# DaLi-Jack/G4Splat

Hardware: AMD Instinct MI355X
Metric: rasterized Gaussians/s fwd+bwd @1600x1200 (higher is better)
Workload: dtype f32

## Files before the change

g4splat_amd/csrc/api.hip:

```cpp
#include <stdarg.h>
#include <stdio.h>
#include <stdlib.h>
#include <string.h>

#include <atomic>
#include <mutex>
#include <vector>

#include "g4s_internal.h"

using namespace g4s;

extern "C" int g4s_knn_launch_internal(int P, const float* points, float* meanDists, char* workspace, hipStream_t s);
extern "C" void g4s_maps_launch_internal(int fwd, int W, int H, float depth_ratio, const float* allmap, const float* wvt,
                                         const float* fpt, float* cam, float* const* outs, const float* surf_depth_in,
                                         const float* const* grads, float* g_allmap, hipStream_t s);

namespace {
thread_local char t_err[512] = "";
}

namespace g4s {
void clear_error() { t_err[0] = 0; }
int fail(int code, const char* fmt, ...) {
// ... 459 lines not shown
}

extern "C" int g4s_rasterizer_forward_presized(
    char* geom_buffer, size_t geom_bytes, char* binning_buffer, size_t binning_bytes, char* image_buffer, size_t image_bytes,
    int instance_capacity, uint32_t* status_dev, int P, int D, int M, const float* background, int width, int height,
    const float* means3D, const float* shs, const float* sh_rest, const float* colors_precomp, const float* opacities,
    const float* scales, float scale_modifier, const float* rotations, const float* transMat_precomp,
    const float* viewmatrix, const float* projmatrix, const float* cam_pos, float tan_fovx, float tan_fovy,
    float* out_color, float* out_others, int* radii, int debug, void* stream) {
    t_err[0] = 0;
    if (instance_capacity < 0 || !status_dev) return fail(G4S_ERR_INVALID_ARGUMENT, "capacity must be >= 0 and status_dev non-NULL");
    if (!geom_buffer || !binning_buffer || !image_buffer) return fail(G4S_ERR_INVALID_ARGUMENT, "state buffers must not be NULL");
    FixedChunk g{geom_buffer, geom_bytes}, b{binning_buffer, binning_bytes}, im{image_buffer, image_bytes};
    DECLARE_FORWARD_CALL(c);
    c.capacity = instance_capacity; c.status_dev = status_dev;
    c.geometry = {fixed_chunk_cb, &g}; c.binning = {fixed_chunk_cb, &b}; c.image = {fixed_chunk_cb, &im};
    c.shs = shs; c.shs_rest = M > 1 ? sh_rest : nullptr; c.colors_precomp = colors_precomp;
    const int rc = rasterizer_forward_impl(c);
    return rc < 0 ? rc : G4S_OK;
}

extern "C" size_t g4s_rasterizer_backward_workspace(int P, int R) {
    (void)P;
    return align_up((size_t)(R > 0 ? R : 1) * GRAD_STRIDE * 4) + 256;
}

static int rasterizer_backward_impl(const BackwardCall& c) {
    hipStream_t stream = (hipStream_t)c.stream;
    const int P = c.P, M = c.M, R = c.R, debug = c.debug;
    t_err[0] = 0;
    if (P < 0 || R < 0 || c.width <= 0 || c.height <= 0) return fail(G4S_ERR_INVALID_ARGUMENT, "bad sizes");
    if (P == 0) return G4S_OK;
    if (!c.geom_buffer || !c.image_buffer || (R > 0 && !c.binning_buffer))
        return fail(G4S_ERR_INVALID_ARGUMENT, "state buffers must not be NULL");
    if (!c.dL_dpix || !c.dL_depths || !c.dL_dmean2D || !c.dL_dopacity || !c.dL_dcolor || !c.dL_dmean3D ||
        !c.dL_dscale || !c.dL_drot || (M > 0 && !c.dL_dsh) || (c.shs_rest && M > 1 && !c.dL_dsh_rest))
        return fail(G4S_ERR_INVALID_ARGUMENT, "NULL gradient pointer");
    if (c.workspace_bytes < g4s_rasterizer_backward_workspace(P, R) || !c.workspace)
        return fail(G4S_ERR_INVALID_ARGUMENT, "workspace too small");
    if (misaligned(c.rotations, 16) || misaligned(c.scales, 8) || misaligned(c.dL_drot, 16) || misaligned(c.dL_dscale, 8))
        return fail(G4S_ERR_INVALID_ARGUMENT, "rotations/dL_drot must be 16-byte, scales/dL_dscale 8-byte aligned");

    const FrameGeom FG = frame_geom(c.width, c.height);
    const int tiles = FG.tiles;
    const GeomLayout GL = geom_layout((size_t)P);
    const BinLayout BL = bin_layout((size_t)R);
    const ImgLayout IL = img_layout((size_t)c.width * c.height, (size_t)tiles);
    char* geom = align_ptr(c.geom_buffer);
    char* img = align_ptr(c.image_buffer);
    const float* rec = (const float*)(geom + GL.rec);
    const int* const radii = c.radii ? c.radii : (const int*)(geom + GL.internal_radii);
    float* grad_inst = (float*)align_ptr(c.workspace);

    uint32_t* hot_count = (uint32_t*)(img + IL.hot_count);
    uint32_t* hot_list = (uint32_t*)(img + IL.hot_list);
    uint8_t* rec_flag = nullptr;
    bool sh_prezeroed = false;
    if (R > 0) {
        char* bin = align_ptr(c.binning_buffer);
        rec_flag = (uint8_t*)(bin + BL.rec_flag);
        BlendBwdArgs bb{};
        bb.W = c.width; bb.H = c.height; bb.tiles_x = FG.tiles_x; bb.tiles_y = FG.tiles_y;
        bb.ranges = (const uint32_t*)(img + IL.ranges);
        uint32_t* tile_order_bwd = (uint32_t*)(img + IL.tile_order_bwd);
        launch_tile_order(tiles, (const uint32_t*)(img + IL.tile_depth), tile_order_bwd, stream, hot_count);
        bb.tile_order = opt(OPT_BWD_FWD_ORDER) ? (const uint32_t*)(img + IL.tile_order) : tile_order_bwd;
        bb.entries = (const uint64_t*)(bin + (FG.entries_in_b ? BL.ent_b : BL.ent_a));
        bb.rec = rec; bb.bg = c.background;
        bb.final_T = (const float*)(img + IL.final_T);
        bb.n_contrib = (const uint32_t*)(img + IL.n_contrib);
        bb.qhit = (const uint8_t*)(bin + BL.qhit);
        bb.dL_dpix = c.dL_dpix; bb.dL_depths = c.dL_depths; bb.grad_inst = grad_inst; bb.rec_flag = rec_flag;
        bb.n_slots = (uint32_t)R;
        const long long avg_list = (long long)R / (tiles > 0 ? tiles : 1);
        const long long outlier = 4 * avg_list > BWD_HOT_THRESHOLD ? 4 * avg_list : BWD_HOT_THRESHOLD;
        const int hot_override = opt(OPT_BWD_HOT_THRESHOLD);
        bb.hot_threshold = hot_override != G4S_OPTION_UNSET ? hot_override
                           : (tiles <= BWD_FOUR_WAVE_MAX_TILES ? -1 : (int)(outlier < 0x7fffffff ? outlier : 0x7fffffff));
        bb.hot_count = hot_count; bb.hot_list = hot_list;
        if (bb.hot_threshold >= 0 && M > 0 && !opt(OPT_NO_SIDE_ZERO) && !c.accumulate) {
            float* zb[2] = {c.dL_dsh, c.dL_dsh_rest};
            const size_t zn[2] = {(size_t)P * (c.dL_dsh_rest ? 1 : M) * 3, c.dL_dsh_rest ? (size_t)P * (M - 1) * 3 : 0};
            bool ok = true;
            for (int z = 0; z < 2; z++) ok = ok && (zn[z] == 0 || (!misaligned(zb[z], 16) && (zn[z] >> 2) < 0x80000000ull));
            if (ok) {
                for (int z = 0; z < 2; z++) {
                    if (zn[z] == 0) continue;
                    bb.zero_base[z] = zb[z]; bb.zero_quads[z] = (uint32_t)(zn[z] >> 2); bb.zero_tail[z] = (uint32_t)(zn[z] & 3);
                }
                sh_prezeroed = true;
            }
        }
        { ProfScope ps(PF_BLEND_BWD, stream); launch_blend_bwd(bb, stream); }
        CHECK_LAUNCH("blend_bwd");
    }

    const float focal_y = c.height / (2.0f * c.tan_fovy);
    const float focal_x = c.width / (2.0f * c.tan_fovx);
    PreprocessBwdArgs pb{};
    pb.P = P; pb.D = c.D; pb.M = M;
    pb.W = (int)(focal_x * c.tan_fovx * 2);
    pb.H = (int)(focal_y * c.tan_fovy * 2);
    pb.means3D = c.means3D; pb.scales = c.scales; pb.rotations = c.rotations; pb.shs = c.shs;
    pb.transMat_precomp = c.transMat_precomp; pb.colors_precomp = c.colors_precomp;
    pb.viewmatrix = c.viewmatrix; pb.projmatrix = c.projmatrix; pb.campos = c.campos;
    pb.radii = radii; pb.rec = rec; pb.clamped = (const uint8_t*)(geom + GL.clamped); pb.grad_inst = grad_inst;
    pb.rec_flag = rec_flag; pb.n_slots = (uint32_t)R;
    pb.frame_W = c.width; pb.frame_H = c.height; pb.scale_modifier = c.scale_modifier;
    pb.shs_rest = c.shs_rest; pb.dL_dsh_rest = c.dL_dsh_rest; pb.sh_prezeroed = sh_prezeroed;
    pb.accumulate = c.accumulate;
    pb.view_stats = c.view_stats;
    const g4s_packed_rows* const packed = c.packed;
    if (packed != nullptr && packed->rows != nullptr) {
        if (c.accumulate) return fail(G4S_ERR_INVALID_ARGUMENT, "packed rows: only the first view of a batch (first_view != 0) can write them");
        if (!packed->block_offs || packed->capacity < 0 || c.shs == nullptr)
            return fail(G4S_ERR_INVALID_ARGUMENT, "packed rows: block_offs must not be NULL, capacity >= 0, colours from SH");
        pb.packed_rows = packed->rows; pb.packed_block_offs = packed->block_offs;
        pb.packed_capacity = (uint32_t)(packed->capacity < 0xFFFFFFFFll ? packed->capacity : 0xFFFFFFFFll);
    }
    if (c.after_event) HIP_TRY(hipStreamWaitEvent(stream, (hipEvent_t)c.after_event, 0));
    pb.sh_vec16 = (c.shs != nullptr && c.shs_rest == nullptr && M == 16 && !misaligned(c.shs, 16) && !misaligned(c.dL_dsh, 16));
    pb.dL_dmean2D = c.dL_dmean2D; pb.dL_dnormal = c.dL_dnormal; pb.dL_dopacity = c.dL_dopacity; pb.dL_dcolor = c.dL_dcolor;
    pb.dL_dmean3D = c.dL_dmean3D; pb.dL_dtransMat = c.dL_dtransMat; pb.dL_dsh = c.dL_dsh; pb.dL_dscale = c.dL_dscale;
    pb.dL_drot = c.dL_drot;
    { ProfScope ps(PF_PREPROCESS_BWD, stream); launch_preprocess_bwd(pb, stream); }
    CHECK_LAUNCH("preprocess_bwd");
    return G4S_OK;
}

extern "C" int g4s_rasterizer_backward(
// ... 407 lines not shown
```

g4splat_amd/csrc/binning.hip:

```cpp
#include "g4s_internal.h"
#include "g4s_device.h"

namespace g4s {


template <typename K>
__device__ __forceinline__ uint32_t radix_digit(K key, uint32_t base, int shift, uint32_t mask) {
    return (uint32_t)((K)(key - (K)base) >> shift) & mask;
}

template <typename K, int ITEMS, int BITS>
__global__ void __launch_bounds__(256) radix_hist_kernel(const K* __restrict__ keys, int n, int shift, uint32_t mask,
                                                         uint32_t* __restrict__ hist, int nblocks,
                                                         const uint32_t* __restrict__ d_n,
                                                         const uint32_t* __restrict__ key_base) {
    constexpr int BINS = 1 << BITS;
    __shared__ uint32_t h[BINS];
    constexpr int TK = 256 * ITEMS;
    const int block = (int)blockIdx.x;
    if (d_n != nullptr) {
        n = (int)*d_n;
        nblocks = (n + TK - 1) / TK;
        if (block >= nblocks) return;
    }
// ... 470 lines not shown
    } else {
#pragma unroll
        for (int k = 0; k < 4; k++) e[k] = entries[i0 + k < R ? i0 + k : R - 1];
    }
    uint32_t prev = i0 > 0 ? entry_tile(entries[i0 - 1]) : 0xFFFFFFFFu;
#pragma unroll
    for (int k = 0; k < 4; k++) {
        const int i = i0 + k;
        if (i >= R) break;
        const uint32_t cur = entry_tile(e[k]);
        if (i == 0) {
            ranges[2 * cur] = 0;
        } else if (cur != prev) {
            ranges[2 * prev + 1] = (uint32_t)i;
            ranges[2 * cur] = (uint32_t)i;
        }
        if (i == R - 1) ranges[2 * cur + 1] = (uint32_t)R;
        prev = cur;
    }
}

constexpr int ORDER_BUCKETS = 2048;
__global__ void __launch_bounds__(1024) tile_order_kernel(int tiles, const uint32_t* __restrict__ ranges,
                                                          uint32_t* __restrict__ order, uint32_t* __restrict__ zero_word) {
    __shared__ uint32_t hist[ORDER_BUCKETS];
    __shared__ uint32_t wsum[16];
    const int t = (int)threadIdx.x;
    if (t == 0 && zero_word != nullptr) *zero_word = 0u;
    for (int i = t; i < ORDER_BUCKETS; i += 1024) hist[i] = 0;
    __syncthreads();
    auto bucket = [](uint32_t n) {
        const uint32_t b = n >> 2;
        return (uint32_t)(ORDER_BUCKETS - 1) - (b < (uint32_t)(ORDER_BUCKETS - 1) ? b : (uint32_t)(ORDER_BUCKETS - 1));
    };
    for (int i = t; i < tiles; i += 1024) atomicAdd(&hist[bucket(ranges[2 * i + 1] - ranges[2 * i])], 1u);
    __syncthreads();
    const uint32_t h0 = hist[2 * t], h1 = hist[2 * t + 1];
    const uint32_t inc = wave_incl_scan_u32(h0 + h1);
    if ((t & 63) == 63) wsum[t >> 6] = inc;
    __syncthreads();
    uint32_t base = 0;
    for (int w = 0; w < (t >> 6); w++) base += wsum[w];
    const uint32_t ex = base + inc - (h0 + h1);
    __syncthreads();
    hist[2 * t] = ex;
    hist[2 * t + 1] = ex + h0;
    __syncthreads();
    for (int i = t; i < tiles; i += 1024) order[atomicAdd(&hist[bucket(ranges[2 * i + 1] - ranges[2 * i])], 1u)] = (uint32_t)i;
}
void launch_tile_order(int tiles, const uint32_t* ranges, uint32_t* tile_order, hipStream_t s, uint32_t* zero_word) {
    hipLaunchKernelGGL(tile_order_kernel, dim3(1), dim3(1024), 0, s, tiles, ranges, tile_order, zero_word);
}

void launch_tile_ranges(int R, const uint64_t* entries, uint32_t* ranges, hipStream_t s, const uint32_t* d_n) {
    if (R <= 0) return;
    hipLaunchKernelGGL(tile_ranges_kernel, dim3((R + 1023) / 1024), dim3(256), 0, s, R, entries, ranges, d_n);
}

}
```

g4splat_amd/csrc/blend.hip:

```cpp
#include "g4s_internal.h"
#include "g4s_device.h"

#ifndef G4S_FWD_PAIRS
#define G4S_FWD_PAIRS 4
#endif

namespace g4s {

__device__ __forceinline__ uint32_t quads_in_box(const float4 q5, uint32_t kx0, uint32_t ky0) {
    const uint32_t x0 = __float_as_uint(q5.x), x1 = __float_as_uint(q5.y), yw = __float_as_uint(q5.w);
    const uint32_t y0 = yw & 0xFFFFu, y1 = yw >> 16;
    const uint32_t cols = (kx0 >= x0 && kx0 <= x1 ? 1u : 0u) | (kx0 + 1 >= x0 && kx0 + 1 <= x1 ? 2u : 0u);
    const uint32_t rows = (ky0 >= y0 && ky0 <= y1 ? 1u : 0u) | (ky0 + 1 >= y0 && ky0 + 1 <= y1 ? 2u : 0u);
    return ((rows & 1u) ? cols : 0u) | ((rows & 2u) ? cols << 2 : 0u);
}

__device__ __forceinline__ bool quad_misses_region(const float4 q0, const float4 q6, const float4 q7, float qx, float qy) {
    const float x1 = qx + 7.0f, y1 = qy + 7.0f;
    const float ddx = fmaxf(fmaxf(qx - q0.x, q0.x - x1), 0.0f), ddy = fmaxf(fmaxf(qy - q0.y, q0.y - y1), 0.0f);
    if (ddx * ddx + ddy * ddy <= q7.z) return false;
    if (q7.x == 0.0f) return false;
    const float ux = q6.z, uy = q6.w, ia = q7.x, ib = q7.y;
    const float ax0 = qx - q6.x, ax1 = x1 - q6.x, ay0 = qy - q6.y, ay1 = y1 - q6.y;
    if (ax0 <= 0.0f && ax1 >= 0.0f && ay0 <= 0.0f && ay1 >= 0.0f) return false;
// ... 202 lines not shown
        a.out_others[pix_id + 3 * N] = st.N1;
        a.out_others[pix_id + 4 * N] = st.N2;
        a.out_others[pix_id + 5 * N] = st.median_depth;
        a.out_others[pix_id + 6 * N] = st.distortion;
    }
}

void launch_blend_fwd(const BlendFwdArgs& a, hipStream_t s) {
    hipLaunchKernelGGL(blend_fwd_kernel, dim3(a.tiles_x * a.tiles_y), dim3(256), 0, s, a);
}


constexpr int BWD_BATCH = 64;

struct BwdPixel {
    float A2, D2, C2, nTfbg;
    uint32_t last_c, median_c;
    float dpx0, dpx1, dpx2, dL_ddepth, dL_daccum, dn0, dn1, dn2, dL_dmedian;
    float T, V_rec, last_dL_dT;
};

__device__ __forceinline__ float fast_rcp(float x) { return __builtin_amdgcn_rcpf(x); }

constexpr int BWD1_BATCH = 48;
struct BwdPixelLite {
    uint32_t last_c;
    float dpx0, dpx1, dpx2, dL_ddepth, dL_daccum, dn0, dn1, dn2;
    float T, V_rec, last_dL_dT;
};
__device__ __forceinline__ void blend_bwd_tile(const BlendBwdArgs& a) {
    __shared__ float4 s_rec[BLEND_QUADS][BWD1_BATCH];
    __shared__ float4 s_cst[256];
    __shared__ float2 s_med[256];

    const int tile = (int)a.tile_order[blockIdx.x];
    const int tile_x = tile % a.tiles_x, tile_y = tile / a.tiles_x;
    const int lane = (int)threadIdx.x;
    const size_t N = (size_t)a.W * a.H;

    const uint32_t r0 = a.ranges[2 * tile], r1 = a.ranges[2 * tile + 1];
    const int n = (int)(r1 - r0);
    if (n == 0) return;

    const int tx0 = tile_x * TILE, ty0 = tile_y * TILE;
    const int px0 = tx0 + (lane & 7), py0 = ty0 + (lane >> 3);
    const float bg0 = a.bg[0], bg1 = a.bg[1], bg2 = a.bg[2];
// ... 22 lines not shown
            x.dn1 = a.dL_depths[pix_id + 3 * N];
            x.dn2 = a.dL_depths[pix_id + 4 * N];
            dL_dmedian = a.dL_depths[pix_id + 5 * N];
            dL_dreg = a.dL_depths[pix_id + 6 * N];
        }
        s_cst[q * 64 + lane] = make_float4((1 - T_final) * dL_dreg, 2.0f * final_D * dL_dreg, final_D2 * dL_dreg,
                                           -T_final * ((bg0 * x.dpx0 + bg1 * x.dpx1) + bg2 * x.dpx2));
        s_med[q * 64 + lane] = make_float2(__uint_as_float(median_c), dL_dmedian);
        x.T = T_final;
        max_last = max(max_last, x.last_c);
    }
    const float mscale = FAR_N / (FAR_N - NEAR_N);
    const float dmd_k = (FAR_N * NEAR_N) / (FAR_N - NEAR_N);
    const bool row_writer = (lane & 15) == 15;
    const int row = lane >> 4;
    const bool lane_b3 = (lane & 8) != 0, lane_b2 = (lane & 4) != 0, quad_writer = (lane & 3) == 0;
    const int term_of_lane = 4 * row + quad_term(lane);

    const int n_live = __builtin_amdgcn_readfirstlane((int)wave_max_u32(max_last));
    if (n_live > a.hot_threshold) {
        if (lane == 0) a.hot_list[atomicAdd(a.hot_count, 1u)] = (uint32_t)tile;
        return;
    }

    for (int hi = n_live; hi > 0; hi -= BWD1_BATCH) {
        const int m = imin_(BWD1_BATCH, hi);
        __syncthreads();
        uint32_t qmask = 0;
        uint32_t slot_l = 0;
        bool nolp_l = false;
        if (lane < m) {
            const uint32_t pos_l = (uint32_t)(hi - 1 - lane);
            qmask = a.qhit[r0 + pos_l];
        }
        if (qmask != 0) {
            const uint32_t pos_l = (uint32_t)(hi - 1 - lane);
            const uint64_t e = a.entries[r0 + pos_l];
            const float4* r = reinterpret_cast<const float4*>(a.rec) + (size_t)entry_idx(e) * REC_QUADS;
            float4 rq[BLEND_QUADS];
#pragma unroll
            for (int i = 0; i < BLEND_QUADS; i++) rq[i] = r[i];
            const float4 q0 = rq[0];
            nolp_l = (__float_as_uint(q0.w) & REC_AFFINE) != 0;
#pragma unroll
            for (int i = 0; i < BLEND_QUADS; i++) s_rec[i][lane] = rq[i];
            slot_l = __float_as_uint(q0.z) + instance_number(__float_as_uint(q0.w), __float_as_uint(reinterpret_cast<const float*>(r)[31]),
// ... 96 lines not shown
                                    dlz = fmaf(dpx_, ky, -(dpy_ * kx));
                        gt0 -= dkx;
                        gt1 -= dky;
                        gt2 -= dkz;
                        gt3 -= dlx;
                        gt4 -= dly;
                        gt5 -= dlz;
                        gt6 += fmaf(pxf, dkx, fmaf(pyf, dlx, dL_dz * e.sx));
                        gt7 += fmaf(pxf, dky, fmaf(pyf, dly, dL_dz * e.sy));
                        gt8 += fmaf(pxf, dkz, fmaf(pyf, dlz, dL_dz));
                    } else {
                        const float c2 = dL_dG * (G * FILTER_INV_SQUARE);
                        glp0 = fmaf(c2, e.dx, glp0);
                        glp1 = fmaf(c2, e.dy, glp1);
                        gt8 += dL_dz;
                        asm volatile("v_mov_b32 %0, 1.0" : "+v"(lowpass));
                    }
                    }
                    gop = fmaf(G, dL_dalpha, gop);
                }
            }
            {
                const uint32_t slot = (uint32_t)__builtin_amdgcn_readlane((int)slot_l, j);
                float t[16] = {gc0, gc1, gc2, gn0, gn1, gn2, gt0, gt1, gt2, gt3, gt4, gt5, gt6, gt7, gt8, gop};
                const float y = wave_sum16_to_quads(t, lane_b3, lane_b2);
                if (slot < a.n_slots) {
                    float* rec = a.grad_inst + (size_t)slot * GRAD_STRIDE;
                    const uint64_t lp_lanes = __ballot(lowpass != 0.0f);
                    uint32_t valid;
                    asm volatile("s_cmp_lg_u64 %1, 0\n\ts_cselect_b32 %0, 3, 1" : "=s"(valid) : "s"(lp_lanes) : "scc");
                    if (quad_writer) {
                        rec[term_of_lane] = y;
                        a.rec_flag[slot] = (uint8_t)valid;
                    }
                    if (valid & 2u) {
                        const float r4 = wave_sum4_to_rows(glp0, glp1, 0.0f, 0.0f);
                        if (row_writer) rec[16 + row] = r4;
                    }
                }
            }
        }
    }
}

__global__ void __launch_bounds__(64) __attribute__((amdgpu_waves_per_eu(4, 4))) blend_bwd_kernel(BlendBwdArgs a) {
    blend_bwd_tile(a);
    const uint32_t lane = threadIdx.x, first = blockIdx.x * 64 + lane, stride = gridDim.x * 64;
#pragma unroll
    for (int z = 0; z < 2; z++) {
        float4* b = reinterpret_cast<float4*>(a.zero_base[z]);
        if (b == nullptr) continue;
        const uint32_t nq = a.zero_quads[z];
        for (uint32_t i = first; i < nq; i += stride) b[i] = make_float4(0.f, 0.f, 0.f, 0.f);
        if (blockIdx.x == 0 && lane < a.zero_tail[z]) reinterpret_cast<float*>(b + nq)[lane] = 0.0f;
    }
}

constexpr int HOT_PART = 20;

__global__ void __launch_bounds__(256) blend_bwd_hot_kernel(BlendBwdArgs a) {
    __shared__ float4 s_rec[BLEND_QUADS][BWD_BATCH];
    __shared__ uint32_t s_slot[BWD_BATCH];
    __shared__ uint32_t s_q[BWD_BATCH];
    __shared__ float s_part[4][BWD_BATCH][HOT_PART];
    __shared__ unsigned long long s_lp[4];
    __shared__ uint32_t s_max[2][4];

    const int wv = (int)(threadIdx.x >> 6), lane = (int)(threadIdx.x & 63);
    const size_t N = (size_t)a.W * a.H;
    const bool all_tiles = a.hot_threshold < 0;
    const uint32_t n_hot = all_tiles ? (uint32_t)(a.tiles_x * a.tiles_y) : *a.hot_count;
    const float bg0 = a.bg[0], bg1 = a.bg[1], bg2 = a.bg[2];
    const float mscale = FAR_N / (FAR_N - NEAR_N);
    const float dmd_k = (FAR_N * NEAR_N) / (FAR_N - NEAR_N);
    const bool row_writer = (lane & 15) == 15;
    const int row = lane >> 4;

    for (uint32_t h = blockIdx.x; h < n_hot; h += gridDim.x) {
        const int tile = (int)(all_tiles ? a.tile_order[h] : a.hot_list[h]);
        const int tile_x = tile % a.tiles_x, tile_y = tile / a.tiles_x;
        const uint32_t r0 = a.ranges[2 * tile];
        const int px = tile_x * TILE + (wv & 1) * 8 + (lane & 7), py = tile_y * TILE + (wv >> 1) * 8 + (lane >> 3);
        const float pxf = (float)px, pyf = (float)py;
        BwdPixel x{};
        {
// ... 10 lines not shown
                x.dpx2 = a.dL_dpix[pix_id + 2 * N];
                x.dL_ddepth = a.dL_depths[pix_id + 0 * N];
                x.dL_daccum = a.dL_depths[pix_id + 1 * N];
                x.dn0 = a.dL_depths[pix_id + 2 * N];
                x.dn1 = a.dL_depths[pix_id + 3 * N];
                x.dn2 = a.dL_depths[pix_id + 4 * N];
                x.dL_dmedian = a.dL_depths[pix_id + 5 * N];
                dL_dreg = a.dL_depths[pix_id + 6 * N];
            }
            x.A2 = (1 - T_final) * dL_dreg;
            x.D2 = 2.0f * final_D * dL_dreg;
            x.C2 = final_D2 * dL_dreg;
            x.nTfbg = -T_final * ((bg0 * x.dpx0 + bg1 * x.dpx1) + bg2 * x.dpx2);
            x.T = T_final;
        }
        __syncthreads();
        {
            const uint32_t ml = wave_max_u32(x.last_c), mm = wave_max_u32(x.median_c);
            if (lane == 0) { s_max[0][wv] = ml; s_max[1][wv] = mm; }
        }
        __syncthreads();
        const int n_live = (int)max(max(s_max[0][0], s_max[0][1]), max(s_max[0][2], s_max[0][3]));
        const uint32_t tile_max_median = max(max(s_max[1][0], s_max[1][1]), max(s_max[1][2], s_max[1][3]));

        for (int hi = n_live; hi > 0; hi -= BWD_BATCH) {
            const int m = imin_(BWD_BATCH, hi);
            __syncthreads();
            if (wv == 0) {
                uint32_t qmask = 0;
                if (lane < m) qmask = a.qhit[r0 + (uint32_t)(hi - 1 - lane)];
                if (qmask != 0) {
                    const uint64_t e = a.entries[r0 + (uint32_t)(hi - 1 - lane)];
                    const float4* r = reinterpret_cast<const float4*>(a.rec) + (size_t)entry_idx(e) * REC_QUADS;
                    float4 rq[BLEND_QUADS];
#pragma unroll
                    for (int i = 0; i < BLEND_QUADS; i++) rq[i] = r[i];
                    if (__float_as_uint(rq[0].w) & REC_AFFINE) qmask |= 16u;
#pragma unroll
                    for (int i = 0; i < BLEND_QUADS; i++) s_rec[i][lane] = rq[i];
                    s_slot[lane] = __float_as_uint(rq[0].z) + instance_number(__float_as_uint(rq[0].w), __float_as_uint(reinterpret_cast<const float*>(r)[31]),
                                                                              (uint32_t)tile_x, (uint32_t)tile_y);
                }
                s_q[lane] = qmask;
            }
            __syncthreads();

            const uint32_t qbits = s_q[lane];
            uint64_t todo = __ballot(((qbits >> wv) & 1u) != 0);
            const uint64_t nolp_mask = __ballot((qbits & 16u) != 0);
            uint64_t lp_mask = 0;
            while (todo) {
                const int j = (int)__builtin_ctzll(todo);
                todo &= ~(1ull << j);
                const bool nolp = (nolp_mask >> j) & 1ull;
                const uint32_t general = (uint32_t)__builtin_amdgcn_readfirstlane(nolp ? 0 : 1);
                const uint32_t pos = (uint32_t)(hi - 1 - j);
                const float4 q0 = s_rec[0][j], q1 = s_rec[1][j], q2 = s_rec[2][j], q3 = s_rec[3][j], q4 = s_rec[4][j];
                float g[18];
#pragma unroll
                for (int i = 0; i < 18; i++) {
                    g[i] = 0.0f;
                    asm volatile("" : "+v"(g[i]));
                }
                bool lowpass = false;
                PairEval e;
                const bool pass = eval_pair(nolp, pxf, pyf, q0.x, q0.y, q2.x, q2.y, q2.z, q2.w, q3.x, q3.y, q3.z, q3.w, q4.x, q1.w, e);
// ... 63 lines not shown
                    }
                    }
                    g[15] = fmaf(G, dL_dalpha, g[15]);
                }
                float t[16] = {g[0], g[1], g[2],  g[3],  g[4],  g[5],  g[6],  g[7],
                               g[8], g[9], g[10], g[11], g[12], g[13], g[14], g[15]};
                float r[4];
                wave_sum16_to_rows(t, r);
                float* part = &s_part[wv][j][0];
                if (row_writer) *reinterpret_cast<float4*>(part + 4 * row) = make_float4(r[0], r[1], r[2], r[3]);
                if (__any(lowpass)) {
                    const float r4 = wave_sum4_to_rows(g[16], g[17], 0.0f, 0.0f);
                    if (row_writer && row < 2) part[16 + row] = r4;
                    lp_mask |= 1ull << j;
                }
            }
            if (lane == 0) s_lp[wv] = lp_mask;
            __syncthreads();

            for (int it = (int)threadIdx.x; it < BWD_BATCH * 5; it += 256) {
                const int e = it / 5, c = it - 5 * e;
                const uint32_t qm = s_q[e] & 15u;
                if (qm == 0) continue;
                const uint32_t slot = s_slot[e];
                if (slot >= a.n_slots) continue;
                float* rec = a.grad_inst + (size_t)slot * GRAD_STRIDE;
                if (c < 4) {
                    float4 acc = make_float4(0, 0, 0, 0);
                    bool first = true;
#pragma unroll
                    for (int w = 0; w < 4; w++) {
                        if (!((qm >> w) & 1u)) continue;
                        const float4 v = *reinterpret_cast<const float4*>(&s_part[w][e][4 * c]);
                        if (first) { acc = v; first = false; }
                        else { acc.x += v.x; acc.y += v.y; acc.z += v.z; acc.w += v.w; }
                    }
                    *reinterpret_cast<float4*>(rec + 4 * c) = acc;
                } else {
                    float ax = 0.0f, ay = 0.0f;
                    bool any_lp = false;
#pragma unroll
                    for (int w = 0; w < 4; w++) {
                        if (((qm >> w) & 1u) && ((s_lp[w] >> e) & 1ull)) {
                            ax = any_lp ? ax + s_part[w][e][16] : s_part[w][e][16];
                            ay = any_lp ? ay + s_part[w][e][17] : s_part[w][e][17];
                            any_lp = true;
                        }
                    }
                    if (any_lp) { rec[16] = ax; rec[17] = ay; }
                    a.rec_flag[slot] = any_lp ? 3 : 1;
                }
            }
        }
    }
}

void launch_blend_bwd(const BlendBwdArgs& a, hipStream_t s) {
    const int tiles = a.tiles_x * a.tiles_y;
    const dim3 hot_grid(tiles < 1024 ? tiles : 1024);
    if (a.hot_threshold < 0) {
        hipLaunchKernelGGL(blend_bwd_hot_kernel, hot_grid, dim3(256), 0, s, a);
        return;
    }
    hipLaunchKernelGGL(blend_bwd_kernel, dim3(tiles), dim3(64), 0, s, a);
    hipLaunchKernelGGL(blend_bwd_hot_kernel, hot_grid, dim3(256), 0, s, a);
}

}
```

g4splat_amd/csrc/g4s_internal.h:

```cpp
#pragma once
#include <hip/hip_runtime.h>
#include <stddef.h>
#include <stdint.h>

#include "../../include/g4s_rasterizer.h"

namespace g4s {

constexpr int TILE = 16;
constexpr int REC_FLOATS = 32;
constexpr int REC_QUADS = REC_FLOATS / 4;
constexpr int BLEND_QUADS = 5;
constexpr int GRAD_FLOATS = 18;
constexpr int GRAD_STRIDE = 20;
__host__ __device__ inline void box_quadrants(float lo, float hi, int extent, uint32_t& q0, uint32_t& q1) {
    const float l = ceilf(lo), h = floorf(hi);
    const float top = (float)(extent - 1);
    q0 = 1u;
    q1 = 0u;
    if (!(l <= h) || !(h >= 0.0f) || !(l <= top)) return;
    q0 = (l > 0.0f ? (uint32_t)l : 0u) >> 3;
    q1 = (h < top ? (uint32_t)h : (uint32_t)(extent - 1)) >> 3;
}
constexpr uint32_t CULLED_KEY = 0xFFFFFFFFu;
#ifndef G4S_SORT_ITEMS_U32
#define G4S_SORT_ITEMS_U32 8
#endif
#ifndef G4S_SORT_ITEMS_U64
#define G4S_SORT_ITEMS_U64 16
#endif
constexpr int SORT_ITEMS_U32 = G4S_SORT_ITEMS_U32;
constexpr int SORT_ITEMS_U64 = G4S_SORT_ITEMS_U64;
inline size_t sort_blocks(size_t n, int items) { return (n + (size_t)256 * items - 1) / ((size_t)256 * items); }
constexpr int DEPTH_SORT_LOW_BITS = 27;
constexpr int ENTRY_TILE_SHIFT = 32;
__host__ __device__ inline uint32_t entry_idx(uint64_t e) { return (uint32_t)e; }
__host__ __device__ inline uint32_t entry_tile(uint64_t e) { return (uint32_t)(e >> ENTRY_TILE_SHIFT); }
// ... 59 lines not shown
    L.hist = c.take((size_t)256 * (sort_blocks(R, SORT_ITEMS_U64) + 1) * 4);
    L.bin_total = c.take(256 * 4);
    L.qhit = c.take((R ? R : 1));
    L.rec_flag = c.take((R ? R : 1));
    L.bytes = c.off + 256;
    return L;
}
inline ImgLayout img_layout(size_t N, size_t tiles) {
    ImgLayout L{};
    WorkspaceCursor c;
    L.ranges = c.take(tiles * 8);
    L.final_T = c.take(N * 3 * 4);
    L.n_contrib = c.take(N * 2 * 4);
    L.tile_order = c.take(tiles * 4);
    L.tile_depth = c.take(tiles * 8);
    L.tile_order_bwd = c.take(tiles * 4);
    L.hot_count = c.take(256);
    L.hot_list = c.take(tiles * 4);
    L.bytes = c.off + 256;
    return L;
}
inline char* align_ptr(char* p) { return (char*)align_up((size_t)p); }

void clear_error();
int fail(int code, const char* fmt, ...);
int finish(hipError_t e, const char* what);


struct PreprocessArgs {
    int P, D, M, W, H, tiles_x, tiles_y;
    uint32_t* ref_block_sums;
    uint32_t* idx_block_sums;
    uint32_t* vis_block_sums;
    uint32_t* key_min_blocks;
    uint32_t* key_max_blocks;
    const float *means3D, *scales, *rotations, *opacities, *shs, *transMat_precomp, *colors_precomp;
    const float *viewmatrix, *projmatrix, *cam_pos;
    float scale_modifier;
    bool sh_vec16;
    bool no_fastpath;
    const float* shs_rest;
    float* rec;
    uint8_t* clamped;
    uint32_t* tiles_touched;
    uint2* tight_rect;
    int* radii;
// ... 6 lines not shown
                         uint32_t* hist, uint32_t* bin_total, hipStream_t s, const uint32_t* d_n = nullptr);
int radix_sort_depth_low(uint32_t* keys_a, uint32_t* keys_b, uint32_t* vals_a, uint32_t* vals_b, int n, uint32_t* hist,
                         uint32_t* bin_total, hipStream_t s, const uint32_t* d_n, const uint32_t* key_min);
int radix_sort_depth_top(uint32_t* keys_a, uint32_t* keys_b, uint32_t* vals_a, uint32_t* vals_b, int n, int cur,
                         uint32_t* hist, uint32_t* bin_total, hipStream_t s, const uint32_t* d_n, const uint32_t* key_min);
int radix_sort_u64_keys(uint64_t* a, uint64_t* b, int n, int begin_bit, int end_bit, uint32_t* hist,
                        uint32_t* bin_total, hipStream_t s, const uint32_t* d_n = nullptr);

void launch_count_scan(int P, const uint32_t* gidx_sorted, const uint32_t* tiles_touched, uint32_t* block_sums,
                       uint32_t* block_offs, uint32_t* rank_local, uint32_t* total, int nblocks, hipStream_t s,
                       const uint32_t* d_n = nullptr);
void launch_scan_totals(const uint32_t* idx_block_sums, uint32_t* idx_block_offs, const uint32_t* ref_block_sums,
                        const uint32_t* vis_block_sums, uint32_t* vis_block_offs, uint32_t* total, int nblocks,
                        uint32_t* zero_ptr, int zero_words, hipStream_t s, uint32_t capacity = 0xFFFFFFFFu,
                        uint32_t* host_out = nullptr, uint32_t* status_out = nullptr,
                        const uint32_t* key_min_blocks = nullptr, const uint32_t* key_max_blocks = nullptr);
void launch_slots_and_compact(int P, const uint32_t* tiles_touched, const uint32_t* idx_block_offs, float* rec,
                              const uint32_t* depth_keys, const uint32_t* vis_block_offs, uint32_t* keys_out,
                              uint32_t* idx_out, int nblocks, hipStream_t s);
void launch_emit(int V, uint32_t R_b, int tiles_x, const uint32_t* gidx_sorted, const uint32_t* block_offs,
                 int nblocks_v, const uint32_t* rank_local, const uint2* tight_rect, uint64_t* entries,
                 uint8_t* qhit, uint8_t* rec_flag, hipStream_t s, const uint32_t* d_counts);
void launch_tile_ranges(int R, const uint64_t* entries, uint32_t* ranges, hipStream_t s, const uint32_t* d_n = nullptr);
void launch_tile_order(int tiles, const uint32_t* ranges, uint32_t* tile_order, hipStream_t s, uint32_t* zero_word = nullptr);

struct BlendFwdArgs {
    int W, H, tiles_x, tiles_y;
    const uint32_t* ranges;
    const uint32_t* tile_order;
    const uint64_t* entries;
    const float* rec;
    const float* bg;
    float* final_T;
    uint32_t* n_contrib;
    uint8_t* qhit;
    uint32_t* tile_depth;
    int box_only;
    float* out_color;
    float* out_others;
};
void launch_blend_fwd(const BlendFwdArgs& a, hipStream_t s);

struct BlendBwdArgs {
    int W, H, tiles_x, tiles_y;
    const uint32_t* ranges;
    const uint32_t* tile_order;
    const uint64_t* entries;
    const float* rec;
    const float* bg;
    const float* final_T;
    const uint32_t* n_contrib;
    const uint8_t* qhit;
    const float* dL_dpix;
    const float* dL_depths;
    float* grad_inst;
    uint8_t* rec_flag;
    uint32_t n_slots;
    int hot_threshold;
    uint32_t* hot_count;
    uint32_t* hot_list;
    float* zero_base[2];
    uint32_t zero_quads[2];
    uint32_t zero_tail[2];
};
constexpr int BWD_HOT_THRESHOLD = 2048;
constexpr int BWD_FOUR_WAVE_MAX_TILES = 768;
void launch_blend_bwd(const BlendBwdArgs& a, hipStream_t s);

struct PreprocessBwdArgs {
    int P, D, M, W, H;
    int frame_W, frame_H;
    float scale_modifier;
    const float *means3D, *scales, *rotations, *shs, *transMat_precomp, *colors_precomp;
    const float *viewmatrix, *projmatrix, *campos;
    const int* radii;
    const float* rec;
    const uint8_t* clamped;
    const float* grad_inst;
    const uint8_t* rec_flag;
    uint32_t n_slots;
    bool sh_vec16;
    const float* shs_rest;
    float* dL_dsh_rest;
    bool sh_prezeroed;
    float* view_stats;
    float* packed_rows;
    const uint32_t* packed_block_offs;
    uint32_t packed_capacity;
    bool accumulate;
    float *dL_dmean2D, *dL_dnormal, *dL_dopacity, *dL_dcolor, *dL_dmean3D, *dL_dtransMat, *dL_dsh, *dL_dscale,
        *dL_drot;
};
void launch_preprocess_bwd(const PreprocessBwdArgs& a, hipStream_t s);

}
```

g4splat_amd/csrc/preprocess.hip:

```cpp
#include "g4s_internal.h"
#include "g4s_device.h"

namespace g4s {

__constant__ float c_SH_C2[5] = {1.0925484305920792f, -1.0925484305920792f, 0.31539156525252005f,
                                 -1.0925484305920792f, 0.5462742152960396f};
__constant__ float c_SH_C3[7] = {-0.5900435899266435f, 2.890611442640554f, -0.4570457994644658f,
                                 0.3731763325901154f,  -0.4570457994644658f, 1.445305721320277f,
                                 -0.5900435899266435f};
#define SH_C0 0.28209479177387814f
#define SH_C1 0.4886025119029199f

__device__ __forceinline__ void compute_transmat(F3 p, float sx, float sy, float mod, const float* R,
                                                 const float* proj, int W, int H, float* T) {
    const float s0 = mod * sx, s1 = mod * sy;
    const float Mrow[3][4] = {{R[0] * s0, R[1] * s0, R[2] * s0, 0.0f},
                              {R[3] * s1, R[4] * s1, R[5] * s1, 0.0f},
                              {p.x, p.y, p.z, 1.0f}};
    const float hw = (float)((float)W / 2.0), cw = (float)((float)(W - 1) / 2.0);
    const float hh = (float)((float)H / 2.0), ch = (float)((float)(H - 1) / 2.0);
#pragma unroll
    for (int r = 0; r < 3; r++) {
        float c[4];
#pragma unroll
// ... 635 lines not shown
        const float4 q0 = rq[0];
        my_off = __float_as_uint(q0.z);
        my_cnt = rect_tiles(__float_as_uint(q0.w));
        if (my_off >= a.n_slots) my_cnt = 0;
        else if (my_cnt > a.n_slots - my_off) my_cnt = a.n_slots - my_off;
    }
    s_off[t] = my_off;
    s_cnt[t] = my_cnt;
    s_vis[t] = visible ? 1 : 0;
    __syncthreads();
    fold_zero_rows(z0, a.P, s_vis);
    fold_zero_rows(z1, a.P, s_vis);
    {
        const int lane = lane_id();
        const int wbase = (t >> 6) * 64;
        const int row = lane >> 4, kk = (lane >> 2) & 3, c = lane & 3;
        constexpr uint32_t FOLD_ROW_MAX = 48;
        uint64_t big = __ballot(my_cnt > FOLD_ROW_MAX);
        while (big) {
            const int j = (int)__builtin_ctzll(big);
            big &= big - 1;
            const uint32_t cnt = (uint32_t)__builtin_amdgcn_readlane((int)my_cnt, j);
            const uint32_t off = (uint32_t)__builtin_amdgcn_readlane((int)my_off, j);
            const float4* base4 = reinterpret_cast<const float4*>(a.grad_inst + (size_t)off * GRAD_STRIDE);
            const uint32_t k16 = (uint32_t)(lane >> 2);
            float4 sA = make_float4(0.f, 0.f, 0.f, 0.f);
            float2 sB = make_float2(0.f, 0.f);
            for (uint32_t k0 = 0; k0 < cnt; k0 += 128) {
                float4 x[8];
                uint8_t f[8];
#pragma unroll
                for (int i = 0; i < 8; i++) {
                    const uint32_t k = k0 + 16 * i + k16;
                    const uint32_t kc = k < cnt ? k : 0u;
                    x[i] = base4[(size_t)kc * (GRAD_STRIDE / 4) + c];
                    f[i] = a.rec_flag[off + kc];
                }
#pragma unroll
                for (int i = 0; i < 8; i++) {
                    const uint32_t k = k0 + 16 * i + k16;
                    if (k < cnt && (f[i] & 1)) { sA.x += x[i].x; sA.y += x[i].y; sA.z += x[i].z; sA.w += x[i].w; }
                    if (k < cnt && (f[i] & 2) && c == 0) {
                        const float2 y = *reinterpret_cast<const float2*>(a.grad_inst + (size_t)(off + k) * GRAD_STRIDE + 16);
                        sB.x += y.x; sB.y += y.y;
                    }
                }
            }
            sA.x += dpp_f32<0x124>(sA.x); sA.y += dpp_f32<0x124>(sA.y); sA.z += dpp_f32<0x124>(sA.z); sA.w += dpp_f32<0x124>(sA.w);
            sA.x += dpp_f32<0x128>(sA.x); sA.y += dpp_f32<0x128>(sA.y); sA.z += dpp_f32<0x128>(sA.z); sA.w += dpp_f32<0x128>(sA.w);
            sA.x += __shfl_xor(sA.x, 16, 64); sA.y += __shfl_xor(sA.y, 16, 64); sA.z += __shfl_xor(sA.z, 16, 64); sA.w += __shfl_xor(sA.w, 16, 64);
            sA.x += __shfl_xor(sA.x, 32, 64); sA.y += __shfl_xor(sA.y, 32, 64); sA.z += __shfl_xor(sA.z, 32, 64); sA.w += __shfl_xor(sA.w, 32, 64);
            sB.x += dpp_f32<0x124>(sB.x); sB.y += dpp_f32<0x124>(sB.y);
            sB.x += dpp_f32<0x128>(sB.x); sB.y += dpp_f32<0x128>(sB.y);
            sB.x += __shfl_xor(sB.x, 16, 64); sB.y += __shfl_xor(sB.y, 16, 64);
            sB.x += __shfl_xor(sB.x, 32, 64); sB.y += __shfl_xor(sB.y, 32, 64);
            float* dst = s_sum + (wbase + j) * K8_SUM_STRIDE;
            if (lane < 4) { dst[4 * lane] = sA.x; dst[4 * lane + 1] = sA.y; dst[4 * lane + 2] = sA.z; dst[4 * lane + 3] = sA.w; }
            if (lane == 0) { dst[16] = sB.x; dst[17] = sB.y; }
        }
        uint64_t vis = __ballot(my_cnt != 0 && my_cnt <= FOLD_ROW_MAX);
        constexpr int U = 3;
        while (vis) {
            int jj[U];
            uint32_t cn[U], of[U];
#pragma unroll
            for (int u = 0; u < U; u++) {
                uint64_t m = vis;
                for (int i = 0; i < row; i++) m &= m - 1;
                jj[u] = m ? (int)__builtin_ctzll(m) : -1;
#pragma unroll
                for (int i = 0; i < 4; i++) vis &= vis - 1;
                cn[u] = jj[u] >= 0 ? s_cnt[wbase + jj[u]] : 0u;
                of[u] = jj[u] >= 0 ? s_off[wbase + jj[u]] : 0u;
            }
            float4 acc[U];
            float2 accB[U];
#pragma unroll
            for (int u = 0; u < U; u++) { acc[u] = make_float4(0.f, 0.f, 0.f, 0.f); accB[u] = make_float2(0.f, 0.f); }
            uint32_t cmax = 0;
#pragma unroll
            for (int u = 0; u < U; u++)
#pragma unroll
                for (int r = 0; r < 4; r++) cmax = max(cmax, (uint32_t)__builtin_amdgcn_readlane((int)cn[u], 16 * r));
            for (uint32_t k0 = 0; k0 < cmax; k0 += 16) {
                float4 x[U][4];
                uint8_t f[U][4];
#pragma unroll
                for (int u = 0; u < U; u++)
#pragma unroll
                    for (int i = 0; i < 4; i++) {
                        const uint32_t k = k0 + 4 * i + kk;
                        f[u][i] = k < cn[u] ? a.rec_flag[of[u] + k] : (uint8_t)0;
                    }
#pragma unroll
                for (int u = 0; u < U; u++) {
                    const float4* base4 = reinterpret_cast<const float4*>(a.grad_inst + (size_t)of[u] * GRAD_STRIDE);
#pragma unroll
                    for (int i = 0; i < 4; i++) {
                        const uint32_t k = k0 + 4 * i + kk;
                        x[u][i] = make_float4(0.f, 0.f, 0.f, 0.f);
                        if (f[u][i] & 1) x[u][i] = base4[(size_t)k * (GRAD_STRIDE / 4) + c];
                    }
                }
#pragma unroll
                for (int u = 0; u < U; u++) {
#pragma unroll
                    for (int i = 0; i < 4; i++) {
                        const uint32_t k = k0 + 4 * i + kk;
                        if (f[u][i] & 1) {
                            acc[u].x += x[u][i].x; acc[u].y += x[u][i].y; acc[u].z += x[u][i].z; acc[u].w += x[u][i].w;
                        }
                        if ((f[u][i] & 2) && c == 0) {
                            const float2 y = *reinterpret_cast<const float2*>(a.grad_inst + (size_t)(of[u] + k) * GRAD_STRIDE + 16);
                            accB[u].x += y.x; accB[u].y += y.y;
                        }
                    }
                }
            }
#pragma unroll
            for (int u = 0; u < U; u++) {
                float4 sA = acc[u];
                float2 sB = accB[u];
                sA.x += dpp_f32<0x124>(sA.x); sA.y += dpp_f32<0x124>(sA.y); sA.z += dpp_f32<0x124>(sA.z); sA.w += dpp_f32<0x124>(sA.w);
                sA.x += dpp_f32<0x128>(sA.x); sA.y += dpp_f32<0x128>(sA.y); sA.z += dpp_f32<0x128>(sA.z); sA.w += dpp_f32<0x128>(sA.w);
                sB.x += dpp_f32<0x124>(sB.x); sB.y += dpp_f32<0x124>(sB.y);
                sB.x += dpp_f32<0x128>(sB.x); sB.y += dpp_f32<0x128>(sB.y);
                if (jj[u] >= 0 && kk == 0) {
                    float* dst = s_sum + (wbase + jj[u]) * K8_SUM_STRIDE;
                    dst[4 * c] = sA.x; dst[4 * c + 1] = sA.y; dst[4 * c + 2] = sA.z; dst[4 * c + 3] = sA.w;
                    if (c == 0) { dst[16] = sB.x; dst[17] = sB.y; }
                }
            }
        }
        if (my_cnt == 0) {
#pragma unroll
            for (int i = 0; i < GRAD_FLOATS; i++) s_sum[t * K8_SUM_STRIDE + i] = 0.0f;
// ... 292 lines not shown
```

Baseline: 268.1 million.

## Compact per-instance gradient records into a dense array indexed via rec_idx

Replaces the slot-indexed 20-float gradient record array with a compacted dense 16-float array plus a separate 2-float lowpass array. Each tile reserves contiguous record positions with an atomic cursor, and a per-slot index maps slots to those positions. The goal is to make blend-backward writes contiguous and to shrink the memory touched when records are sparse. In exchange it adds an atomic per tile, an extra index array, and an indirect gather in the preprocess reduction, which loses the locality of the per-Gaussian contiguous slot range.

```diff
diff --git a/g4splat_amd/csrc/api.hip b/g4splat_amd/csrc/api.hip
--- a/g4splat_amd/csrc/api.hip
+++ b/g4splat_amd/csrc/api.hip
@@ -505,7 +505,7 @@
 
 extern "C" size_t g4s_rasterizer_backward_workspace(int P, int R) {
     (void)P;
-    return align_up((size_t)(R > 0 ? R : 1) * GRAD_STRIDE * 4) + 256;
+    return bwd_workspace_layout((size_t)(R > 0 ? R : 0)).bytes;
 }
 
 static int rasterizer_backward_impl(const BackwardCall& c) {
@@ -519,7 +519,8 @@
     if (!c.dL_dpix || !c.dL_depths || !c.dL_dmean2D || !c.dL_dopacity || !c.dL_dcolor || !c.dL_dmean3D ||
         !c.dL_dscale || !c.dL_drot || (M > 0 && !c.dL_dsh) || (c.shs_rest && M > 1 && !c.dL_dsh_rest))
         return fail(G4S_ERR_INVALID_ARGUMENT, "NULL gradient pointer");
-    if (c.workspace_bytes < g4s_rasterizer_backward_workspace(P, R) || !c.workspace)
+    const BwdWorkspace WL = bwd_workspace_layout((size_t)R);
+    if (c.workspace_bytes < WL.bytes || !c.workspace)
         return fail(G4S_ERR_INVALID_ARGUMENT, "workspace too small");
     if (misaligned(c.rotations, 16) || misaligned(c.scales, 8) || misaligned(c.dL_drot, 16) || misaligned(c.dL_dscale, 8))
         return fail(G4S_ERR_INVALID_ARGUMENT, "rotations/dL_drot must be 16-byte, scales/dL_dscale 8-byte aligned");
@@ -533,7 +534,11 @@
     char* img = align_ptr(c.image_buffer);
     const float* rec = (const float*)(geom + GL.rec);
     const int* const radii = c.radii ? c.radii : (const int*)(geom + GL.internal_radii);
-    float* grad_inst = (float*)align_ptr(c.workspace);
+    char* ws = align_ptr(c.workspace);
+    float* dense = (float*)(ws + WL.dense);
+    float* lowpass = (float*)(ws + WL.lowpass);
+    uint32_t* rec_idx = (uint32_t*)(ws + WL.rec_idx);
+    uint32_t* cursor = (uint32_t*)(ws + WL.cursor);
 
     uint32_t* hot_count = (uint32_t*)(img + IL.hot_count);
     uint32_t* hot_list = (uint32_t*)(img + IL.hot_list);
@@ -546,14 +551,15 @@
         bb.W = c.width; bb.H = c.height; bb.tiles_x = FG.tiles_x; bb.tiles_y = FG.tiles_y;
         bb.ranges = (const uint32_t*)(img + IL.ranges);
         uint32_t* tile_order_bwd = (uint32_t*)(img + IL.tile_order_bwd);
-        launch_tile_order(tiles, (const uint32_t*)(img + IL.tile_depth), tile_order_bwd, stream, hot_count);
+        launch_tile_order(tiles, (const uint32_t*)(img + IL.tile_depth), tile_order_bwd, stream, hot_count, cursor);
         bb.tile_order = opt(OPT_BWD_FWD_ORDER) ? (const uint32_t*)(img + IL.tile_order) : tile_order_bwd;
         bb.entries = (const uint64_t*)(bin + (FG.entries_in_b ? BL.ent_b : BL.ent_a));
         bb.rec = rec; bb.bg = c.background;
         bb.final_T = (const float*)(img + IL.final_T);
         bb.n_contrib = (const uint32_t*)(img + IL.n_contrib);
         bb.qhit = (const uint8_t*)(bin + BL.qhit);
-        bb.dL_dpix = c.dL_dpix; bb.dL_depths = c.dL_depths; bb.grad_inst = grad_inst; bb.rec_flag = rec_flag;
+        bb.dL_dpix = c.dL_dpix; bb.dL_depths = c.dL_depths; bb.dense = dense; bb.lowpass = lowpass;
+        bb.rec_idx = rec_idx; bb.cursor = cursor; bb.rec_flag = rec_flag;
         bb.n_slots = (uint32_t)R;
         const long long avg_list = (long long)R / (tiles > 0 ? tiles : 1);
         const long long outlier = 4 * avg_list > BWD_HOT_THRESHOLD ? 4 * avg_list : BWD_HOT_THRESHOLD;
@@ -587,8 +593,8 @@
     pb.means3D = c.means3D; pb.scales = c.scales; pb.rotations = c.rotations; pb.shs = c.shs;
     pb.transMat_precomp = c.transMat_precomp; pb.colors_precomp = c.colors_precomp;
     pb.viewmatrix = c.viewmatrix; pb.projmatrix = c.projmatrix; pb.campos = c.campos;
-    pb.radii = radii; pb.rec = rec; pb.clamped = (const uint8_t*)(geom + GL.clamped); pb.grad_inst = grad_inst;
-    pb.rec_flag = rec_flag; pb.n_slots = (uint32_t)R;
+    pb.radii = radii; pb.rec = rec; pb.clamped = (const uint8_t*)(geom + GL.clamped); pb.dense = dense; pb.lowpass = lowpass;
+    pb.rec_idx = rec_idx; pb.rec_flag = rec_flag; pb.n_slots = (uint32_t)R;
     pb.frame_W = c.width; pb.frame_H = c.height; pb.scale_modifier = c.scale_modifier;
     pb.shs_rest = c.shs_rest; pb.dL_dsh_rest = c.dL_dsh_rest; pb.sh_prezeroed = sh_prezeroed;
     pb.accumulate = c.accumulate;
diff --git a/g4splat_amd/csrc/binning.hip b/g4splat_amd/csrc/binning.hip
--- a/g4splat_amd/csrc/binning.hip
+++ b/g4splat_amd/csrc/binning.hip
@@ -516,11 +516,13 @@
 
 constexpr int ORDER_BUCKETS = 2048;
 __global__ void __launch_bounds__(1024) tile_order_kernel(int tiles, const uint32_t* __restrict__ ranges,
-                                                          uint32_t* __restrict__ order, uint32_t* __restrict__ zero_word) {
+                                                          uint32_t* __restrict__ order, uint32_t* __restrict__ zero_word,
+                                                          uint32_t* __restrict__ zero_word2) {
     __shared__ uint32_t hist[ORDER_BUCKETS];
     __shared__ uint32_t wsum[16];
     const int t = (int)threadIdx.x;
     if (t == 0 && zero_word != nullptr) *zero_word = 0u;
+    if (t == 1 && zero_word2 != nullptr) *zero_word2 = 0u;
     for (int i = t; i < ORDER_BUCKETS; i += 1024) hist[i] = 0;
     __syncthreads();
     auto bucket = [](uint32_t n) {
@@ -542,8 +544,9 @@
     __syncthreads();
     for (int i = t; i < tiles; i += 1024) order[atomicAdd(&hist[bucket(ranges[2 * i + 1] - ranges[2 * i])], 1u)] = (uint32_t)i;
 }
-void launch_tile_order(int tiles, const uint32_t* ranges, uint32_t* tile_order, hipStream_t s, uint32_t* zero_word) {
-    hipLaunchKernelGGL(tile_order_kernel, dim3(1), dim3(1024), 0, s, tiles, ranges, tile_order, zero_word);
+void launch_tile_order(int tiles, const uint32_t* ranges, uint32_t* tile_order, hipStream_t s, uint32_t* zero_word,
+                       uint32_t* zero_word2) {
+    hipLaunchKernelGGL(tile_order_kernel, dim3(1), dim3(1024), 0, s, tiles, ranges, tile_order, zero_word, zero_word2);
 }
 
 void launch_tile_ranges(int R, const uint64_t* entries, uint32_t* ranges, hipStream_t s, const uint32_t* d_n) {
diff --git a/g4splat_amd/csrc/blend.hip b/g4splat_amd/csrc/blend.hip
--- a/g4splat_amd/csrc/blend.hip
+++ b/g4splat_amd/csrc/blend.hip
@@ -248,6 +248,24 @@
 
 __device__ __forceinline__ float fast_rcp(float x) { return __builtin_amdgcn_rcpf(x); }
 
+__device__ __forceinline__ uint32_t record_block(const uint8_t* __restrict__ qhit, int n_live, int lane, uint32_t* cursor) {
+    uint32_t n_rec = 0;
+    for (int b = 0; b < n_live; b += 256) {
+        uint32_t q[4];
+#pragma unroll
+        for (int i = 0; i < 4; i++) {
+            const int pl = b + 64 * i + lane;
+            q[i] = pl < n_live ? (uint32_t)qhit[pl] : 0u;
+        }
+#pragma unroll
+        for (int i = 0; i < 4; i++) n_rec += (uint32_t)__popcll(__ballot(q[i] != 0));
+    }
+    if (n_rec == 0) return 0u;
+    uint32_t first = 0;
+    if (lane == 0) first = atomicAdd(cursor, n_rec);
+    return (uint32_t)__builtin_amdgcn_readfirstlane((int)first);
+}
+
 constexpr int BWD1_BATCH = 48;
 struct BwdPixelLite {
     uint32_t last_c;
@@ -316,6 +334,7 @@
         if (lane == 0) a.hot_list[atomicAdd(a.hot_count, 1u)] = (uint32_t)tile;
         return;
     }
+    uint32_t rec_pos = record_block(a.qhit + r0, n_live, lane, a.cursor);
 
     for (int hi = n_live; hi > 0; hi -= BWD1_BATCH) {
         const int m = imin_(BWD1_BATCH, hi);
@@ -458,20 +477,23 @@
             }
             {
                 const uint32_t slot = (uint32_t)__builtin_amdgcn_readlane((int)slot_l, j);
+                const uint32_t rpos = rec_pos;
+                rec_pos += 1u;
                 float t[16] = {gc0, gc1, gc2, gn0, gn1, gn2, gt0, gt1, gt2, gt3, gt4, gt5, gt6, gt7, gt8, gop};
                 const float y = wave_sum16_to_quads(t, lane_b3, lane_b2);
-                if (slot < a.n_slots) {
-                    float* rec = a.grad_inst + (size_t)slot * GRAD_STRIDE;
+                if (max(slot, rpos) < a.n_slots) {
+                    float* rec = a.dense + (size_t)rpos * DENSE_REC_FLOATS;
                     const uint64_t lp_lanes = __ballot(lowpass != 0.0f);
                     uint32_t valid;
                     asm volatile("s_cmp_lg_u64 %1, 0\n\ts_cselect_b32 %0, 3, 1" : "=s"(valid) : "s"(lp_lanes) : "scc");
                     if (quad_writer) {
                         rec[term_of_lane] = y;
                         a.rec_flag[slot] = (uint8_t)valid;
+                        a.rec_idx[slot] = rpos;
                     }
                     if (valid & 2u) {
                         const float r4 = wave_sum4_to_rows(glp0, glp1, 0.0f, 0.0f);
-                        if (row_writer) rec[16 + row] = r4;
+                        if (row_writer && row < LOWPASS_FLOATS) a.lowpass[(size_t)rpos * LOWPASS_FLOATS + row] = r4;
                     }
                 }
             }
@@ -497,6 +519,7 @@
 __global__ void __launch_bounds__(256) blend_bwd_hot_kernel(BlendBwdArgs a) {
     __shared__ float4 s_rec[BLEND_QUADS][BWD_BATCH];
     __shared__ uint32_t s_slot[BWD_BATCH];
+    __shared__ uint32_t s_pos[BWD_BATCH];
     __shared__ uint32_t s_q[BWD_BATCH];
     __shared__ float s_part[4][BWD_BATCH][HOT_PART];
     __shared__ unsigned long long s_lp[4];
@@ -553,6 +576,8 @@
         __syncthreads();
         const int n_live = (int)max(max(s_max[0][0], s_max[0][1]), max(s_max[0][2], s_max[0][3]));
         const uint32_t tile_max_median = max(max(s_max[1][0], s_max[1][1]), max(s_max[1][2], s_max[1][3]));
+        uint32_t rec_pos = 0;
+        if (wv == 0) rec_pos = record_block(a.qhit + r0, n_live, lane, a.cursor);
 
         for (int hi = n_live; hi > 0; hi -= BWD_BATCH) {
             const int m = imin_(BWD_BATCH, hi);
@@ -573,6 +598,9 @@
                                                                               (uint32_t)tile_x, (uint32_t)tile_y);
                 }
                 s_q[lane] = qmask;
+                const uint64_t hit = __ballot(qmask != 0);
+                s_pos[lane] = rec_pos + (uint32_t)__popcll(hit & ((1ull << lane) - 1ull));
+                rec_pos += (uint32_t)__popcll(hit);
             }
             __syncthreads();
 
@@ -682,9 +710,9 @@
                 const int e = it / 5, c = it - 5 * e;
                 const uint32_t qm = s_q[e] & 15u;
                 if (qm == 0) continue;
-                const uint32_t slot = s_slot[e];
-                if (slot >= a.n_slots) continue;
-                float* rec = a.grad_inst + (size_t)slot * GRAD_STRIDE;
+                const uint32_t slot = s_slot[e], rpos = s_pos[e];
+                if (slot >= a.n_slots || rpos >= a.n_slots) continue;
+                float* rec = a.dense + (size_t)rpos * DENSE_REC_FLOATS;
                 if (c < 4) {
                     float4 acc = make_float4(0, 0, 0, 0);
                     bool first = true;
@@ -707,8 +735,9 @@
                             any_lp = true;
                         }
                     }
-                    if (any_lp) { rec[16] = ax; rec[17] = ay; }
+                    if (any_lp) *reinterpret_cast<float2*>(a.lowpass + (size_t)rpos * LOWPASS_FLOATS) = make_float2(ax, ay);
                     a.rec_flag[slot] = any_lp ? 3 : 1;
+                    a.rec_idx[slot] = rpos;
                 }
             }
         }
diff --git a/g4splat_amd/csrc/g4s_internal.h b/g4splat_amd/csrc/g4s_internal.h
--- a/g4splat_amd/csrc/g4s_internal.h
+++ b/g4splat_amd/csrc/g4s_internal.h
@@ -12,7 +12,8 @@
 constexpr int REC_QUADS = REC_FLOATS / 4;
 constexpr int BLEND_QUADS = 5;
 constexpr int GRAD_FLOATS = 18;
-constexpr int GRAD_STRIDE = 20;
+constexpr int DENSE_REC_FLOATS = 16;
+constexpr int LOWPASS_FLOATS = 2;
 __host__ __device__ inline void box_quadrants(float lo, float hi, int extent, uint32_t& q0, uint32_t& q1) {
     const float l = ceilf(lo), h = floorf(hi);
     const float top = (float)(extent - 1);
@@ -118,6 +119,28 @@
 }
 inline char* align_ptr(char* p) { return (char*)align_up((size_t)p); }
 
+struct BwdWorkspace {
+    size_t rec_idx;
+    size_t dense;
+    size_t lowpass;
+    size_t cursor;
+    size_t bytes;
+};
+constexpr size_t BWD_WS_FLOOR_SLOT_BYTES = 80;
+inline BwdWorkspace bwd_workspace_layout(size_t R) {
+    BwdWorkspace L{};
+    WorkspaceCursor c;
+    const size_t n = R ? R : 1;
+    L.rec_idx = c.take(n * 4);
+    L.dense = c.take(n * DENSE_REC_FLOATS * 4);
+    L.lowpass = c.take(n * LOWPASS_FLOATS * 4);
+    L.cursor = c.take(4);
+    L.bytes = c.off + 256;
+    const size_t floor_bytes = align_up(n * BWD_WS_FLOOR_SLOT_BYTES) + 256;
+    if (L.bytes < floor_bytes) L.bytes = floor_bytes;
+    return L;
+}
+
 void clear_error();
 int fail(int code, const char* fmt, ...);
 int finish(hipError_t e, const char* what);
@@ -170,7 +193,8 @@
                  int nblocks_v, const uint32_t* rank_local, const uint2* tight_rect, uint64_t* entries,
                  uint8_t* qhit, uint8_t* rec_flag, hipStream_t s, const uint32_t* d_counts);
 void launch_tile_ranges(int R, const uint64_t* entries, uint32_t* ranges, hipStream_t s, const uint32_t* d_n = nullptr);
-void launch_tile_order(int tiles, const uint32_t* ranges, uint32_t* tile_order, hipStream_t s, uint32_t* zero_word = nullptr);
+void launch_tile_order(int tiles, const uint32_t* ranges, uint32_t* tile_order, hipStream_t s, uint32_t* zero_word = nullptr,
+                       uint32_t* zero_word2 = nullptr);
 
 struct BlendFwdArgs {
     int W, H, tiles_x, tiles_y;
@@ -201,7 +225,10 @@
     const uint8_t* qhit;
     const float* dL_dpix;
     const float* dL_depths;
-    float* grad_inst;
+    float* dense;
+    float* lowpass;
+    uint32_t* rec_idx;
+    uint32_t* cursor;
     uint8_t* rec_flag;
     uint32_t n_slots;
     int hot_threshold;
@@ -224,7 +251,9 @@
     const int* radii;
     const float* rec;
     const uint8_t* clamped;
-    const float* grad_inst;
+    const float* dense;
+    const float* lowpass;
+    const uint32_t* rec_idx;
     const uint8_t* rec_flag;
     uint32_t n_slots;
     bool sh_vec16;
diff --git a/g4splat_amd/csrc/preprocess.hip b/g4splat_amd/csrc/preprocess.hip
--- a/g4splat_amd/csrc/preprocess.hip
+++ b/g4splat_amd/csrc/preprocess.hip
@@ -681,26 +681,31 @@
             big &= big - 1;
             const uint32_t cnt = (uint32_t)__builtin_amdgcn_readlane((int)my_cnt, j);
             const uint32_t off = (uint32_t)__builtin_amdgcn_readlane((int)my_off, j);
-            const float4* base4 = reinterpret_cast<const float4*>(a.grad_inst + (size_t)off * GRAD_STRIDE);
+            const float4* dense4 = reinterpret_cast<const float4*>(a.dense);
+            const float2* lowpass2 = reinterpret_cast<const float2*>(a.lowpass);
             const uint32_t k16 = (uint32_t)(lane >> 2);
             float4 sA = make_float4(0.f, 0.f, 0.f, 0.f);
             float2 sB = make_float2(0.f, 0.f);
             for (uint32_t k0 = 0; k0 < cnt; k0 += 128) {
                 float4 x[8];
                 uint8_t f[8];
+                uint32_t id[8];
 #pragma unroll
                 for (int i = 0; i < 8; i++) {
                     const uint32_t k = k0 + 16 * i + k16;
-                    const uint32_t kc = k < cnt ? k : 0u;
-                    x[i] = base4[(size_t)kc * (GRAD_STRIDE / 4) + c];
-                    f[i] = a.rec_flag[off + kc];
+                    f[i] = k < cnt ? a.rec_flag[off + k] : (uint8_t)0;
+                    id[i] = k < cnt ? a.rec_idx[off + k] : 0u;
                 }
 #pragma unroll
                 for (int i = 0; i < 8; i++) {
-                    const uint32_t k = k0 + 16 * i + k16;
-                    if (k < cnt && (f[i] & 1)) { sA.x += x[i].x; sA.y += x[i].y; sA.z += x[i].z; sA.w += x[i].w; }
-                    if (k < cnt && (f[i] & 2) && c == 0) {
-                        const float2 y = *reinterpret_cast<const float2*>(a.grad_inst + (size_t)(off + k) * GRAD_STRIDE + 16);
+                    x[i] = make_float4(0.f, 0.f, 0.f, 0.f);
+                    if (f[i] & 1) x[i] = dense4[(size_t)id[i] * (DENSE_REC_FLOATS / 4) + c];
+                }
+#pragma unroll
+                for (int i = 0; i < 8; i++) {
+                    if (f[i] & 1) { sA.x += x[i].x; sA.y += x[i].y; sA.z += x[i].z; sA.w += x[i].w; }
+                    if ((f[i] & 2) && c == 0) {
+                        const float2 y = lowpass2[id[i]];
                         sB.x += y.x; sB.y += y.y;
                     }
                 }
@@ -744,33 +749,33 @@
             for (uint32_t k0 = 0; k0 < cmax; k0 += 16) {
                 float4 x[U][4];
                 uint8_t f[U][4];
+                uint32_t id[U][4];
 #pragma unroll
                 for (int u = 0; u < U; u++)
 #pragma unroll
                     for (int i = 0; i < 4; i++) {
                         const uint32_t k = k0 + 4 * i + kk;
                         f[u][i] = k < cn[u] ? a.rec_flag[of[u] + k] : (uint8_t)0;
+                        id[u][i] = k < cn[u] ? a.rec_idx[of[u] + k] : 0u;
                     }
+                const float4* dense4 = reinterpret_cast<const float4*>(a.dense);
 #pragma unroll
                 for (int u = 0; u < U; u++) {
-                    const float4* base4 = reinterpret_cast<const float4*>(a.grad_inst + (size_t)of[u] * GRAD_STRIDE);
 #pragma unroll
                     for (int i = 0; i < 4; i++) {
-                        const uint32_t k = k0 + 4 * i + kk;
                         x[u][i] = make_float4(0.f, 0.f, 0.f, 0.f);
-                        if (f[u][i] & 1) x[u][i] = base4[(size_t)k * (GRAD_STRIDE / 4) + c];
+                        if (f[u][i] & 1) x[u][i] = dense4[(size_t)id[u][i] * (DENSE_REC_FLOATS / 4) + c];
                     }
                 }
 #pragma unroll
                 for (int u = 0; u < U; u++) {
 #pragma unroll
                     for (int i = 0; i < 4; i++) {
-                        const uint32_t k = k0 + 4 * i + kk;
                         if (f[u][i] & 1) {
                             acc[u].x += x[u][i].x; acc[u].y += x[u][i].y; acc[u].z += x[u][i].z; acc[u].w += x[u][i].w;
                         }
                         if ((f[u][i] & 2) && c == 0) {
-                            const float2 y = *reinterpret_cast<const float2*>(a.grad_inst + (size_t)(of[u] + k) * GRAD_STRIDE + 16);
+                            const float2 y = reinterpret_cast<const float2*>(a.lowpass)[id[u][i]];
                             accB[u].x += y.x; accB[u].y += y.y;
                         }
                     }
```

Result: slower. 254.2 million (-5.2%).
